# leonsick/depthg

Hardware: AMD Instinct MI355X
Metric: correlation-loss steps/sec at B=32,C=384,28x28 (fwd+bwd, per-GPU batch 32) (higher is better)
Workload: dtype bf16 (feats) / f16 (code) MFMA inputs, f32 accumulate

## Files before the change

### depthg_amd/csrc/dg_api_corr.hip

```cpp
#include "dg_api.h"
#include "dg_corr_args.h"
#include "dg_taps.h"

static unsigned long long* g_prof_span = nullptr;
extern "C" int dg_prof_main_span(void* span) { g_prof_span = static_cast<unsigned long long*>(span); return DG_OK; }

enum class Prep { Small, Dense, General };
enum class Sampler { Plane, ChannelLast };
enum class MainKernel { Small, Corr2, CorrMain };
enum class Depth { None, Job, GsBlocks, GsOwnLaunch };
enum class Hist { Rows, Blobs };
enum class Masks { None, Sampled, DenseRaw, DenseSplit };

struct PairSet {
    int rop;
    int op;
    int neg;
    bool mapped;
    float shift;
    int slot_loss, slot_cd;
    float fin_scale;
    int gidx, csel, dest;
    float factor;
};
// ... 23 lines not shown
    float shift_depth;
    float inv_numel;
    float grad_f, grad_fn;
    int blob, blob_off_c;
    PairSet ps[DG_MAX_NEG + 2];
    Operand ops[DG_MAX_NEG + 2];
    bool gr_on;
    int gr_nkeys, gr_cpb, gr_blocks_per_image;
    int8_t gr_key[DG_MAX_JOBS], gr_first[DG_MAX_JOBS];
    int32_t gr_nblk[DG_MAX_JOBS];
    size_t nhwc_f[2], nhwc_c[2];
    size_t rows_f[DG_MAX_NEG + 2], rows_c[DG_MAX_NEG + 2];
    size_t op[DG_MAX_NEG + 2], inv[DG_MAX_NEG + 2], colpart[DG_MAX_NEG + 2], bbar[DG_MAX_NEG + 2];
    size_t ccolpart[DG_MAX_NEG + 2], csum[DG_MAX_NEG + 2], bsplit[DG_MAX_NEG + 2];
    size_t rvec[DG_MAX_NEG + 2], rimg[DG_MAX_NEG + 2];
    size_t nz, nzsum;
    size_t dRA[DG_MAX_NEG + 3], dRB[DG_MAX_NEG + 2];
    size_t part[DG_MAX_NEG + 3];
    size_t comb[2], scratch_out, taps, gbuf[DG_MAX_NEG + 2];
    size_t ticket;
    size_t maskbits[DG_MAX_NEG + 2];
    size_t clo[2];
    size_t gr_list, gr_count, gr_rank;
    size_t dRA2[DG_MAX_NEG + 2], dRBs[DG_MAX_NEG + 2], dRB2[DG_MAX_NEG + 2][2], dRBm[DG_MAX_NEG + 2], part4, om;
    size_t total;

    bool small() const { return prep == Prep::Small; }
    bool dense() const { return prep == Prep::Dense; }
    bool plane() const { return sampler == Sampler::Plane; }
    bool has_masks() const { return masks != Masks::None; }
    bool depth_in_gs() const { return depth_run == Depth::GsBlocks || depth_run == Depth::GsOwnLaunch; }
    bool dense_masks() const { return masks == Masks::DenseRaw || masks == Masks::DenseSplit; }
    bool intra_symmetric() const { return !pointwise || fold; }
    const int64_t* batch_map(int k, const int64_t* perms) const {
        return k < 0 ? nullptr : reinterpret_cast<const int64_t*>(reinterpret_cast<uintptr_t>(perms) + (size_t)k * B * sizeof(int64_t));
    }
    const int64_t* map_of(int t, const int64_t* perms) const { return batch_map(ps[t].mapped ? ps[t].neg : -1, perms); }
};

static inline float* f32(char* ws, size_t off) { return reinterpret_cast<float*>(ws + off); }

#define FOLD_STASH_OFF (5 * 1024)

static void plan_tables(const dg_corr_desc* d, Plan& p) {
    const double numel = (double)p.B * p.P * p.P;
    p.inv_numel = (float)(1.0 / numel);
// ... 125 lines not shown
    for (int i = 0; i < 2; ++i) p.comb[i] = take(B * p.Ppad * p.KD * 4);
    p.scratch_out = take(DG_OUT_COUNT * 4);
    p.taps = take(2 * B * dg_taps_record_bytes(p.hc * p.wc, p.P));
    for (int t = 0; t < p.T; ++t) p.gbuf[t] = p.grad ? take(B * (size_t)(p.Ppad / 32) * (p.Ppad / 32) * 2048) : 0;
    p.ticket = take(256);
    const bool xmask = rows && !p.small() && p.grad && plain_zero_clamp && p.Ppad <= 256 && p.rf == 4;
    const bool xmask_dense = (d->flags & DG_EXACT_MASKS) && ident && p.grad && plain_zero_clamp &&
                             p.KF == 384 && p.KD == 96 && p.D <= 80 && p.Ppad >= 160 && p.B <= 64;
    if ((d->flags & DG_EXACT_MASKS) && p.grad && (d->flags & DG_ZERO_CLAMP) && !xmask && !xmask_dense && !p.small())
        return fail(DG_ERR_UNSUPPORTED, "DG_EXACT_MASKS: exact clamp masks exist on small sample grids (always on there) and on the dense "
                                        "identity grid with C <= 384 (padded to 384), D <= 80, P >= 160, B <= 64, zero_clamp without stabalize");
    p.masks = xmask ? Masks::Sampled : (!xmask_dense ? Masks::None : (p.pointwise ? Masks::DenseSplit : Masks::DenseRaw));
    for (int t = 0; t < p.T; ++t) p.maskbits[t] = take(p.has_masks() ? B * (size_t)(p.Ppad / 32) * p.Ppad * 4 : 0);
    p.main = p.small() ? MainKernel::Small
                       : (p.grad && dg_corr2_shape_supported(p.KF, p.KD, p.D, p.lo, p.hi, p.Ppad, p.B) ? MainKernel::Corr2 : MainKernel::CorrMain);
    static const bool fold_on = [] { const char* e = getenv("DG_FOLD_INTRA"); return !(e && e[0] == '0'); }();
    p.fold = fold_on && p.main == MainKernel::Corr2 && p.pointwise && !xmask;
    p.half = p.main == MainKernel::Corr2 && ident && p.N * p.B <= 512 && p.S == p.h && p.S == p.w;
    p.depth_run = (!p.depth || p.small()) ? Depth::None : (!p.grad ? Depth::Job : (p.dense_masks() ? Depth::GsOwnLaunch : Depth::GsBlocks));
    for (int i = 0; i < 2; ++i) p.clo[i] = take(p.masks == Masks::DenseSplit ? B * (size_t)(p.Ppad / 32) * p.KD * 64 : 0);
    p.gr_list = take((size_t)DG_MAX_JOBS * B * DG_GR_CAP * 4);
    p.gr_count = take((size_t)DG_MAX_JOBS * B * 4);
    p.gr_rank = take((size_t)DG_MAX_JOBS * B * 2);
    {
        const bool sg = p.small() && p.grad, two = sg && p.pointwise;
        const size_t gt = B * p.Ppad * p.KD * 4;
        for (int t = 0; t < p.T; ++t) {
            p.dRA2[t] = take(two ? gt : 0);
            p.dRBs[t] = take(sg && p.nsplit == 2 ? gt : 0);
            for (int k = 0; k < 2; ++k) p.dRB2[t][k] = take(two && k < p.nsplit ? gt : 0);
            p.dRBm[t] = take(sg && t >= 2 && (p.pointwise || p.nsplit == 2) ? gt : 0);
        }
        p.part4 = take(p.small() ? (size_t)(p.T + 1) * B * p.nsplit * 16 : 0);
        p.om = take(p.small() ? (size_t)(p.T + 1) * 4 : 0);
    }
    if (intra_feats) {
        const int x = p.xop = p.T;
        p.nhwc_x = take(rows ? 0 : B * HW * p.C4 * 4);
        p.rows_f[x] = take(want_rows ? B * p.P * frow : 0); p.rows_c[x] = p.rows_c[0];
        p.op[x] = take(B * (p.Ppad / 32) * (size_t)p.blob);
        p.inv[x] = take(B * p.Ppad * 4);
        p.colpart[x] = take(B * (size_t)(p.Ppad / 32) * p.KF * 4);
        p.bbar[x] = take(B * p.KF * 4);
        p.bsplit[x] = take(B * 2 * p.KF * 2);
        p.ccolpart[x] = take(B * (size_t)(p.Ppad / 32) * p.KD * 4);
        p.csum[x] = take(B * p.KD * 4);
// ... 345 lines not shown
    return DG_OK;
}

static int fwd_colmeans(Fwd& c) {
    const Plan& p = c.p;
    const DgCorrArgs& a = c.a;
    DgColmeanArgs m;
    memset(&m, 0, sizeof(m));
    m.nops = p.nopx(); m.B = p.B; m.P = p.P; m.Ppad = p.Ppad; m.KF = p.KF; m.KD = p.KD;
    for (int o = 0; o < p.nopx(); ++o) {
        m.colpart[o] = p.pointwise ? f32(c.ws, p.colpart[o]) : nullptr; m.bbar[o] = f32(c.ws, p.bbar[o]);
        m.bsplit[o] = reinterpret_cast<__bf16*>(c.ws + p.bsplit[o]);
        m.ngroups[o] = p.Ppad / 32;
        m.ccolpart[o] = f32(c.ws, p.ccolpart[o]); m.csum[o] = f32(c.ws, p.csum[o]);
    }
    m.zero_word = p.depth_in_gs() ? reinterpret_cast<unsigned int*>(c.ws + p.ticket) : nullptr;
    m.zero_words9 = a.wctr;
    if (p.gr_on) {
        m.gr.nh = p.T; m.gr.nkeys = p.gr_nkeys; m.gr.B = p.B;
        for (int t = 0; t < p.T; ++t) { m.gr.sidx[t] = p.map_of(t, c.perms); m.gr.key[t] = p.gr_key[t]; }
        m.gr.list = reinterpret_cast<int32_t*>(c.ws + p.gr_list); m.gr.count = reinterpret_cast<int32_t*>(c.ws + p.gr_count);
        m.gr.rank = reinterpret_cast<int16_t*>(c.ws + p.gr_rank);
    }
    if (p.dense() && p.pointwise) {
        m.dc.code[0] = c.code; m.dc.code[1] = c.code_pos;
        for (int o = 0; o < 2; ++o) { m.dc.blob[o] = c.ws + p.op[o]; m.dc.inv_norm[o] = f32(c.ws, p.inv[o]); m.dc.ccolpart[o] = f32(c.ws, p.ccolpart[o]); }
        m.dc.B = p.B; m.dc.D = p.D; m.dc.KF = p.KF; m.dc.KD = p.KD; m.dc.h = p.h; m.dc.w = p.w; m.dc.P = p.P; m.dc.Ppad = p.Ppad;
        if (p.masks == Masks::DenseSplit) { m.dc.clo[0] = c.ws + p.clo[0]; m.dc.clo[1] = c.ws + p.clo[1]; }
    }
    if (c.split) {
        DgColmeanArgs ms = m;
        ms.zsel = 1; m.zsel = 2;
        DG_HIP(c.side->hand_over(0));
        DG_HIP(dg_launch_colmean(ms, c.side->stream()));
    }
    DG_HIP(dg_launch_colmean(m, c.stream));
    return DG_OK;
}

static int fwd_cd_mask3(Fwd& c) {
    const Plan& p = c.p;
    DgCdMask3Args m;
    memset(&m, 0, sizeof(m));
    m.opR = c.ws + p.op[0]; m.loR = c.ws + p.clo[0];
    for (int t = 0; t < p.T; ++t) {
        m.opS[t] = c.ws + p.op[p.ps[t].op]; m.loS[t] = c.ws + p.clo[p.ps[t].op]; m.sidx[t] = p.map_of(t, c.perms);
// ... 228 lines not shown
static int corr_backward_impl(const dg_corr_desc* desc, const float* grad_scalars, const float* grad_total, const float* coords1,
                              const float* coords2, const int64_t* perms, float* grad_code, float* grad_code_pos,
                              void* workspace, size_t workspace_bytes, dg_stream_t stream_) {
    Plan p{};
    int rc = make_plan(desc, p);
    if (rc != DG_OK) return rc;
    if (!p.grad) return fail(DG_ERR_INVALID, "dg_corr_backward needs a descriptor with DG_NEED_GRAD (as used in forward)");
    if (!coords1 || !coords2 || !grad_code || !grad_code_pos || !workspace) return fail(DG_ERR_INVALID, "null pointer");
    if (p.N > 0 && !perms) return fail(DG_ERR_INVALID, "perms is null with n_neg=%d", p.N);
    if (workspace_bytes < p.total) return fail(DG_ERR_WORKSPACE, "workspace %zu < required %zu bytes", workspace_bytes, p.total);
    char* ws = static_cast<char*>(workspace);
    DgScatterArgs s;
    memset(&s, 0, sizeof(s));
    ScatterFill fill{s, ws};
    if (p.small()) scatter_sources_small(p, perms, fill);
    else scatter_sources_blobs(p, perms, fill);
    if (p.depth) fill.add(p.dRA[p.T], nullptr, 3, 0, 2.0f * p.grad_f, 0, 1);
    s.coords1 = coords1; s.coords2 = coords2; s.gscal = grad_scalars; s.gtot = grad_total;
    s.wtot[0] = desc->w_intra; s.wtot[1] = desc->w_inter; s.wtot[2] = desc->w_neg; s.wtot[3] = desc->w_depth;
    s.comb[0] = f32(ws, p.comb[0]); s.comb[1] = f32(ws, p.comb[1]);
    s.taps = ws + p.taps;
    s.xop = ws + p.op[0]; s.xinv = f32(ws, p.inv[0]); s.blob_bytes = p.blob; s.blob_off_c = p.blob_off_c;
    s.xinv_dest[0] = f32(ws, p.inv[0]); s.xinv_dest[1] = p.nops > 1 ? f32(ws, p.inv[1]) : nullptr;
    s.out[0] = grad_code; s.out[1] = grad_code_pos;
    s.B = p.B; s.D = p.D; s.DP = p.KD; s.h = p.hc; s.w = p.wc; s.S = p.S; s.Sh = p.Sh; s.P = p.P; s.Ppad = p.Ppad;
    if ((size_t)p.hc * p.wc > 4096) return fail(DG_ERR_UNSUPPORTED, "code map %dx%d too large for the gradient gather (max 4096 pixels)", p.hc, p.wc);
    s.DC = 8;
    s.dense = p.dense() ? 1 : 0;
    s.taps_ready = p.dense() ? 0 : 1;
    DG_HIP(dg_launch_scatter(s, static_cast<hipStream_t>(stream_)));
    return DG_OK;
}

extern "C" int dg_corr_backward(const dg_corr_desc* desc, const float* grad_scalars, const float* coords1,
                                const float* coords2, const int64_t* perms, float* grad_code, float* grad_code_pos,
                                void* workspace, size_t workspace_bytes, dg_stream_t stream_) {
    if (!grad_scalars) return fail(DG_ERR_INVALID, "null pointer");
    return corr_backward_impl(desc, grad_scalars, nullptr, coords1, coords2, perms, grad_code, grad_code_pos, workspace,
                              workspace_bytes, stream_);
}

extern "C" int dg_corr_backward_total(const dg_corr_desc* desc, const float* grad_total, const float* coords1,
                                      const float* coords2, const int64_t* perms, float* grad_code, float* grad_code_pos,
                                      void* workspace, size_t workspace_bytes, dg_stream_t stream_) {
    if (!grad_total) return fail(DG_ERR_INVALID, "null pointer");
    return corr_backward_impl(desc, nullptr, grad_total, coords1, coords2, perms, grad_code, grad_code_pos, workspace,
// ... 125 lines not shown
```

### depthg_amd/csrc/dg_corr_args.h

```cpp
#pragma once
#include "dg_device.h"

__host__ __device__ inline int dg_perm32(int pl) {
    int s = pl >> 4, u = (pl >> 3) & 1, hh = (pl >> 2) & 1, v = pl & 3;
    return (2 * s + hh) * 8 + 4 * u + v;
}

#ifndef DG_F_IG
#define DG_F_IG 4
#endif
__host__ __device__ inline int dg_f_off(int q, int g) {
    constexpr int IG = DG_F_IG;
    return ((g / IG) * 32 + q) * (IG * 16) + (((g % IG) ^ ((q / (16 / IG)) % IG)) * 16);
}

struct DgBlob {
    int GF, GD, KD;
    int off_c, off_p, bytes;
    __host__ __device__ DgBlob(int KF, int KD_) : GF(KF / 8), GD(KD_ / 8), KD(KD_) {
        off_c = 32 * GF * 16;
        off_p = off_c + GD * 32 * 16;
        bytes = off_p + 4 * KD * 16;
    }
    __host__ __device__ int f(int q, int g) const { return dg_f_off(q, g); }
// ... 1 lines not shown
    __host__ __device__ int p(int d, int cc) const { return off_p + (cc * KD + d) * 16; }
};

template <int NKF, int NKD>
struct BlobT {
    static constexpr int KF = NKF * 16, KD = NKD * 16, GF = KF / 8, GD = KD / 8;
    static constexpr int OFF_C = 32 * GF * 16;
    static constexpr int OFF_P = OFF_C + GD * 32 * 16;
    static constexpr int BYTES = OFF_P + 4 * KD * 16;
    static constexpr int CHUNKS = BYTES / 1024;
    static constexpr int CHUNK_C0 = OFF_C / 1024;
    static constexpr int CHUNK_P0 = OFF_P / 1024;
    static_assert(BYTES % 1024 == 0 && OFF_C % 1024 == 0 && OFF_P % 1024 == 0, "blob parts must be KiB multiples");
    static_assert(GF % 16 == 0, "swizzle needs 16-granule groups");
};

__host__ __device__ inline size_t dg_gtile_off(int p, int d, int DP) {
    const int q = p & 31;
    return ((size_t)(p >> 5) * (DP >> 5) + (d >> 5)) * 1024 + (q >> 3) * 256 + ((d & 31) + 32 * ((q >> 2) & 1)) * 4 + (q & 3);
}

#define DG_XROWS_LDS (4 * 33 * 16)
template <int NDF>
__device__ __forceinline__ void dg_load_code_rows(const char* Cp, char* T, int lane, _Float16 (&x)[NDF][16]) {
        const int r = lane & 31, h = lane >> 5;
    i32x4 raw[NDF][2];
#pragma unroll
    for (int f = 0; f < NDF; ++f)
#pragma unroll
        for (int k = 0; k < 2; ++k) raw[f][k] = *reinterpret_cast<const i32x4*>(Cp + f * 2048 + k * 1024 + lane * 16);
#pragma unroll
    for (int f = 0; f < NDF; ++f) {
#pragma unroll
        for (int k = 0; k < 2; ++k) {
            const int L = k * 64 + lane;
            *reinterpret_cast<i32x4*>(T + ((L >> 5) * 33 + (L & 31)) * 16) = raw[f][k];
        }
#pragma unroll
        for (int i = 0; i < 16; ++i) {
            const int q = (i & 3) + 8 * (i >> 2) + 4 * h;
            x[f][i] = *reinterpret_cast<const _Float16*>(T + ((r >> 3) * 33 + q) * 16 + (r & 7) * 2);
        }
    }
}

enum { DG_JOB_HELPER = 0, DG_JOB_DEPTH = 1 };

struct DgJob {
    const char* Rop;
    const char* Sop;
    const float* rvec;
    const float* rimg;
    const uint32_t* maskbits;
    const float* nzR;
    const float* nzS;
    const float* RcInv;
    const float* Scsum;
    const int64_t* ridx;
    const int64_t* sidx;
    float* dR;
    float* part;
    float* out_cd;
    float* out_loss;
    uint16_t* Gout;
    float shift;
    int32_t kind;
// ... 251 lines not shown
    const int B = g.B;
    int src[DG_MAX_JOBS];
#pragma unroll
    for (int j = 0; j < DG_MAX_JOBS; ++j) {
        const bool mine = j < g.nh && g.key[j] == key && lane < B;
        const int64_t* sidx = mine ? g.sidx[j] : nullptr;
        src[j] = mine ? (sidx ? (int)sidx[lane] : lane) : -1;
    }
    int cnt = 0;
#pragma unroll
    for (int j = 0; j < DG_MAX_JOBS; ++j) {
        const bool hit = src[j] == m;
        const unsigned long long mask = __ballot(hit);
        if (hit) {
            const int rk = cnt + __popcll(mask & ((1ull << lane) - 1ull));
            g.rank[j * B + lane] = (int16_t)(rk < 32767 ? rk : 32767);
            if (rk < DG_GR_CAP) g.list[(key * B + m) * DG_GR_CAP + rk] = j | (lane << 8);
        }
        cnt += __popcll(mask);
    }
    if (lane == 0) g.count[key * B + m] = cnt < DG_GR_CAP ? cnt : DG_GR_CAP;
}

struct DgColmeanArgs {
    const float* colpart[DG_MAX_NEG + 2];
    float* bbar[DG_MAX_NEG + 2];
    __bf16* bsplit[DG_MAX_NEG + 2];
    const float* ccolpart[DG_MAX_NEG + 2];
    float* csum[DG_MAX_NEG + 2];
    int32_t ngroups[DG_MAX_NEG + 2];
    int32_t nops, B, P, Ppad, KF, KD;
    unsigned int* zero_word;
    unsigned int* zero_words9;
    DgGroupArgs gr;
    DgDenseCodeArgs dc;
    int32_t zsel;
};

struct DgRowmeanJob {
    const char* A;
    const float* bbar;
    const __bf16* bsplit;
    const int64_t* aidx;
    const int64_t* bidx;
    float* rvec;
    float* rimg;
};
struct DgRowmeanArgs {
    DgRowmeanJob jobs[DG_MAX_NEG + 2];
    int32_t njobs, B, P, Ppad, KF, KD;
    const float* abar;
    const char* xA;
    const float* xabar;
    char* stash;
    int32_t stash_off;
    const float* cs_part[2];
    float* cs_out[2];
// ... 14 lines not shown
#define DG_MAX_SCATTER 48
struct DgScatterArgs {
    DgScatterSrc src[DG_MAX_SCATTER];
    int32_t nsrc;
    const float* coords1;
    const float* coords2;
    const float* gscal;
    const float* gtot;
    float wtot[4];
    float* comb[2];
    char* taps;
    const char* xop;
    const float* xinv;
    const float* xinv_dest[2];
    int32_t blob_bytes, blob_off_c;
    float* out[2];
    int32_t B, D, DP, h, w, S, Sh, P, Ppad, DC;
    int32_t dense;
    int8_t craw[2][DG_MAX_SCATTER / 2], cfin[2][DG_MAX_SCATTER / 2];
    int8_t ncraw[2], ncfin[2];
    int8_t crawh[2][DG_MAX_SCATTER / 2], cfinh[2][DG_MAX_SCATTER / 2];
    int8_t ncrawh[2], ncfinh[2];
    int32_t routed_half;
    int32_t taps_ready;
    int32_t naxpy;
    float* axo[DG_MAX_NEG + 2];
    const float* axd[DG_MAX_NEG + 2];
    const float* axd2[DG_MAX_NEG + 2];
    const float* axs[DG_MAX_NEG + 2];
    const float* axs2[DG_MAX_NEG + 2];
    const float* axf[DG_MAX_NEG + 2];
};

__device__ __forceinline__ float dg_src_factor(const DgScatterSrc& q) { return q.dfac ? q.factor * q.dfac[0] : q.factor; }
__device__ __forceinline__ float dg_gscal(const DgScatterArgs& a, int i) {
    return a.gscal ? a.gscal[i] + a.gscal[DG_OUT_TOTAL] * a.wtot[i] : a.gtot[0] * a.wtot[i];
}

struct DgGsJob {
    const uint16_t* G;
    const char* Rop;
    const char* Sop;
    const float* ScInv;
    const int64_t* ridx;
    const int64_t* sidx;
    float* dS;
// ... 66 lines not shown
```

### depthg_amd/csrc/dg_post.hip

```cpp
#include "dg_device.h"
#include "dg_corr_args.h"
#include "dg_taps.h"
#include <cstdlib>

typedef const float __attribute__((address_space(1)))* gfloat_p;


#define DG_LOAD_GS(a, gs)                                                                                   \
    float gs[4];                                                                                            \
    {                                                                                                       \
        const bool vec_ = (a).gscal != nullptr;                                                             \
        const float gt_ = vec_ ? (a).gscal[DG_OUT_TOTAL] : (a).gtot[0];                                     \
        const float g0_ = vec_ ? (a).gscal[0] : 0.f, g1_ = vec_ ? (a).gscal[1] : 0.f;                       \
        const float g2_ = vec_ ? (a).gscal[2] : 0.f, g3_ = vec_ ? (a).gscal[3] : 0.f;                       \
        gs[0] = g0_ + gt_ * (a).wtot[0]; gs[1] = g1_ + gt_ * (a).wtot[1];                                  \
        gs[2] = g2_ + gt_ * (a).wtot[2]; gs[3] = g3_ + gt_ * (a).wtot[3];                                  \
    }
__device__ __forceinline__ float dg_pick(const float (&gs)[4], int i) { return i == 0 ? gs[0] : (i == 1 ? gs[1] : (i == 2 ? gs[2] : gs[3])); }

template <int NDF>
__global__ __launch_bounds__(64 * NDF) void k_grad_combine(const DgScatterArgs a) {
    const int rt = blockIdx.x, n = blockIdx.y, dest = blockIdx.z;
    const int lane = threadIdx.x & 63, r = lane & 31, h = lane >> 5, DP = NDF * 32;
    const int d = __builtin_amdgcn_readfirstlane((int)threadIdx.x >> 6);
    if (dest >= 2) {
        const int j = dest - 2;
        const size_t off = ((size_t)n * (a.Ppad >> 5) + rt) * (32 * DP) + d * 1024 + lane * 4;
        const float f = a.axf[j] ? a.axf[j][0] : 0.f;
// ... 68 lines not shown
            const float inv = rr < a.P ? a.xinv[(size_t)n * a.Ppad + rr] : 0.f;
            v[i] = (v[i] - (float)x[0][i] * t) * inv;
        }
    }
    add_sources(a.cfin[dest], a.ncfin[dest]);
    if (ok) {
        float* out = a.comb[dest] + tile_off;
#pragma unroll
        for (int g = 0; g < 4; ++g) {
            const f32x4 t = {v[4 * g], v[4 * g + 1], v[4 * g + 2], v[4 * g + 3]};
            *reinterpret_cast<f32x4*>(out + g * 256) = t;
        }
    }
}

#ifndef COMB_HB_HM
#define COMB_HB_HM 4
#endif
#ifndef COMB_HB
#define COMB_HB 4
#endif
#define COMB_MAXROUTE 512
template <int NDF, bool HM = false>
__global__ __launch_bounds__(64 * NDF) void k_combine_out(const DgScatterArgs a) {
    const int rt = blockIdx.x, n = blockIdx.y, dest = blockIdx.z;
    const int tid = threadIdx.x, lane = tid & 63, r = lane & 31, h = lane >> 5, DP = NDF * 32;
    const int d = __builtin_amdgcn_readfirstlane(tid >> 6);
    __shared__ __attribute__((aligned(16))) char xs[NDF][DG_XROWS_LDS];
    __shared__ float part[NDF][32];
    __shared__ float stage[NDF][32 * 33];
    __shared__ const float* rl_p[COMB_MAXROUTE];
    __shared__ float rl_w[COMB_MAXROUTE];
    __shared__ int rl_cnt, wcnt[NDF], rsrc[DG_MAX_SCATTER];
    DG_LOAD_GS(a, gs)
    int nr = 0;
    for (int s = 0; s < a.nsrc; ++s)
        if (a.src[s].dest == dest && a.src[s].route != nullptr) { if (tid == 0) rsrc[nr] = s; ++nr; }
    if (tid == 0) rl_cnt = 0;
    __syncthreads();
    for (int i0 = 0; i0 < nr * a.B; i0 += 64 * NDF) {
        const int i = i0 + tid;
        bool hit = false;
        int m = 0, s = 0;
        if (i < nr * a.B) {
            const int rs = i / a.B;
            m = i - rs * a.B; s = rsrc[rs];
            hit = (int)a.src[s].route[m] == n;
        }
        const unsigned long long bal = __ballot(hit);
        if (lane == 0) wcnt[d] = __popcll(bal);
        __syncthreads();
        int base = rl_cnt;
        for (int wv = 0; wv < d; ++wv) base += wcnt[wv];
        if (hit) {
            const int o = base + __popcll(bal & ((1ull << lane) - 1));
            const DgScatterSrc& q = a.src[s];
            if (o < COMB_MAXROUTE) {
                rl_p[o] = q.half ? reinterpret_cast<const float*>(reinterpret_cast<const _Float16*>(q.buf) + (size_t)m * a.Ppad * a.DP) : q.buf + (size_t)m * a.Ppad * a.DP;
                rl_w[o] = dg_src_factor(q) * dg_pick(gs, q.gidx);
            }
        }
        __syncthreads();
        if (tid == 0) {
            int c = rl_cnt;
            for (int wv = 0; wv < NDF; ++wv) c += wcnt[wv];
            rl_cnt = min(c, COMB_MAXROUTE);
        }
        __syncthreads();
    }
    const int cnt = rl_cnt;
    const bool ok = 32 * d + r < a.D;
    const size_t in_img = (size_t)rt * (32 * DP) + lane * 4 + (ok ? d * 1024 : 0);
    const size_t tile_off = (size_t)n * a.Ppad * DP + in_img;
    float v[16];
#pragma unroll
    for (int i = 0; i < 16; ++i) v[i] = 0.f;
    const size_t in_img_h = (size_t)rt * (32 * DP) + lane * 8 + (ok ? d * 1024 : 0);
    constexpr int HB = HM ? COMB_HB_HM : COMB_HB, FB = HM ? 1 : 4;
    float invd[16];
#pragma unroll
    for (int i = 0; i < 16; ++i) {
        const int rr = rt * 32 + (i & 3) + 8 * (i >> 2) + 4 * h;
        invd[i] = (a.xinv_dest[dest] && rr < a.P) ? a.xinv_dest[dest][(size_t)n * a.Ppad + rr] : 0.f;
    }
    const _Float16 __attribute__((address_space(1)))* const hdummy = reinterpret_cast<const _Float16 __attribute__((address_space(1)))*>(reinterpret_cast<uintptr_t>(a.xinv));
    auto add_half4 = [&](const _Float16 __attribute__((address_space(1)))* const (&hb)[HB], const float (&sc)[HB], const bool raw) __attribute__((always_inline)) {
        f16x8 t0[HB], t1[HB];
#pragma unroll
        for (int u = 0; u < HB; ++u) {
            t0[u] = *reinterpret_cast<const f16x8 __attribute__((address_space(1)))*>(hb[u]);
            t1[u] = *reinterpret_cast<const f16x8 __attribute__((address_space(1)))*>(hb[u] + ((ok && hb[u] != hdummy) ? 512 : 0));
        }
#pragma unroll
        for (int u = 0; u < HB; ++u) {
            const bool use = ok && sc[u] != 0.f;
#pragma unroll
            for (int e = 0; e < 8; ++e) {
                v[e] = fmaf(raw ? sc[u] : sc[u] * invd[e], use ? (float)t0[u][e] : 0.f, v[e]);
                v[8 + e] = fmaf(raw ? sc[u] : sc[u] * invd[8 + e], use ? (float)t1[u][e] : 0.f, v[8 + e]);
            }
        }
    };
    auto add_sources_half = [&](const int8_t* list, const int nsrc_, const bool raw) __attribute__((always_inline)) {
        for (int k0 = 0; k0 < nsrc_; k0 += HB) {
            const _Float16 __attribute__((address_space(1)))* hb[HB];
            float sc[HB];
#pragma unroll
            for (int u = 0; u < HB; ++u) {
                const bool live = k0 + u < nsrc_;
                const DgScatterSrc& q = a.src[(int)list[live ? k0 + u : k0]];
                sc[u] = live ? dg_src_factor(q) * dg_pick(gs, q.gidx) : 0.f;
                hb[u] = live ? reinterpret_cast<const _Float16 __attribute__((address_space(1)))*>(reinterpret_cast<uintptr_t>(q.buf)) + (size_t)n * a.Ppad * DP + in_img_h
                             : hdummy;
            }
            add_half4(hb, sc, raw);
        }
    };
    auto add_sources = [&](const int8_t* list, const int nsrc_) __attribute__((always_inline)) {

        for (int k0 = 0; k0 < nsrc_; k0 += FB) {
            f32x4 t[FB][4];
            float sc[FB];
#pragma unroll
            for (int u = 0; u < FB; ++u) {
                const bool live = k0 + u < nsrc_;
                const DgScatterSrc& q = a.src[(int)list[live ? k0 + u : k0]];
                sc[u] = live ? dg_src_factor(q) * dg_pick(gs, q.gidx) : 0.f;
                const float* base = q.buf + tile_off;
#pragma unroll
                for (int g = 0; g < 4; ++g) t[u][g] = *reinterpret_cast<const f32x4*>(base + (ok ? g * 256 : 0));
            }
#pragma unroll
            for (int u = 0; u < FB; ++u) {
                const bool use = ok && k0 + u < nsrc_;
#pragma unroll
                for (int g = 0; g < 4; ++g)
#pragma unroll
                    for (int e = 0; e < 4; ++e) v[4 * g + e] = fmaf(sc[u], use ? t[u][g][e] : 0.f, v[4 * g + e]);
            }
        }
    };
    const int nraw = a.ncraw[dest] + a.ncrawh[dest];
    add_sources(a.craw[dest], a.ncraw[dest]);
    add_sources_half(a.crawh[dest], a.ncrawh[dest], true);
    if (nraw > 0) {
        const char* xb = a.xop + ((size_t)n * (a.Ppad >> 5) + rt) * a.blob_bytes + a.blob_off_c + d * 2048;
        _Float16 x[1][16];
        dg_load_code_rows<1>(xb, xs[d], lane, x);
#pragma unroll
        for (int i = 0; i < 16; ++i) {
            const float t = half_sum((float)x[0][i] * v[i]);
            if (r == 0) part[d][h * 16 + i] = t;
        }
        __syncthreads();
#pragma unroll
        for (int i = 0; i < 16; ++i) {
            float t = part[0][h * 16 + i];
#pragma unroll
            for (int f = 1; f < NDF; ++f) t += part[f][h * 16 + i];
            const int rr = rt * 32 + (i & 3) + 8 * (i >> 2) + 4 * h;
            const float inv = rr < a.P ? a.xinv[(size_t)n * a.Ppad + rr] : 0.f;
            v[i] = (v[i] - (float)x[0][i] * t) * inv;
        }
    }
    add_sources(a.cfin[dest], a.ncfin[dest]);
    add_sources_half(a.cfinh[dest], a.ncfinh[dest], false);
    if (a.routed_half) {
        for (int e0 = 0; e0 < cnt; e0 += HB) {
            const _Float16 __attribute__((address_space(1)))* hb[HB];
            float sc[HB];
#pragma unroll
            for (int k = 0; k < HB; ++k) {
                const int e = min(e0 + k, cnt - 1);
                sc[k] = e0 + k < cnt ? rl_w[e] : 0.f;
                hb[k] = sc[k] != 0.f ? reinterpret_cast<const _Float16 __attribute__((address_space(1)))*>(reinterpret_cast<uintptr_t>(rl_p[e])) + in_img_h : hdummy;
            }
            add_half4(hb, sc, false);
        }
    } else
    for (int e0 = 0; e0 < cnt; e0 += 4) {
        f32x4 u4[4][4];
        float sc[4];
#pragma unroll
        for (int k = 0; k < 4; ++k) {
            const int e = min(e0 + k, cnt - 1);
            sc[k] = e0 + k < cnt ? rl_w[e] : 0.f;
            const gfloat_p sb = (gfloat_p)rl_p[e] + in_img;
#pragma unroll
            for (int g = 0; g < 4; ++g) u4[k][g] = *(const f32x4 __attribute__((address_space(1)))*)(sb + (ok ? g * 256 : 0));
        }
#pragma unroll
        for (int k = 0; k < 4; ++k)
#pragma unroll
            for (int g = 0; g < 4; ++g)
#pragma unroll
                for (int e = 0; e < 4; ++e) v[4 * g + e] = fmaf(sc[k], ok ? u4[k][g][e] : 0.f, v[4 * g + e]);
    }
    float* st = stage[d];
#pragma unroll
    for (int i = 0; i < 16; ++i) st[r * 33 + (i & 3) + 8 * (i >> 2) + 4 * h] = v[i];
    __builtin_amdgcn_fence(__ATOMIC_RELEASE, "workgroup");
    __builtin_amdgcn_wave_barrier();
    __builtin_amdgcn_fence(__ATOMIC_ACQUIRE, "workgroup");
    const int HW = a.h * a.w, p = rt * 32 + r;
    float* out = a.out[dest] + (size_t)n * a.D * HW + p;
#pragma unroll
    for (int it = 0; it < 16; ++it) {
        const int c = 2 * it + h, ch = 32 * d + c;
        if (ch < a.D && p < a.P) out[(size_t)ch * HW] = st[c * 33 + r];
    }
// ... 364 lines not shown
    {
        for (int dest = 0; dest < 2; ++dest) {
            ac.ncraw[dest] = ac.ncfin[dest] = ac.ncrawh[dest] = ac.ncfinh[dest] = 0;
            for (int i = 0; i < a.nsrc; ++i) {
                const DgScatterSrc& q = a.src[i];
                if (q.dest != dest || q.route != nullptr) continue;
                int8_t& cnt = q.half ? (q.raw ? ac.ncrawh[dest] : ac.ncfinh[dest]) : (q.raw ? ac.ncraw[dest] : ac.ncfin[dest]);
                if (cnt >= DG_MAX_SCATTER / 2) return hipErrorInvalidValue;
                (q.half ? (q.raw ? ac.crawh[dest] : ac.cfinh[dest]) : (q.raw ? ac.craw[dest] : ac.cfin[dest]))[cnt++] = (int8_t)i;
            }
        }
        const dim3 cgrid(a.Ppad / 32, a.B, 2);
        {
            int nrouted = 0;
            for (int i = 0; i < a.nsrc; ++i) nrouted += a.src[i].route != nullptr;
            bool any_half = false;
            int routed_h = 0;
            for (int i = 0; i < a.nsrc; ++i) { any_half = any_half || a.src[i].half != 0; routed_h += (a.src[i].route != nullptr && a.src[i].half) ? 1 : 0; }
            if (routed_h != 0 && routed_h != nrouted) return hipErrorInvalidValue;
            ac.routed_half = routed_h != 0 ? 1 : 0;
            const bool one_launch = a.dense && a.S == a.h && a.S == a.w && nrouted * a.B <= COMB_MAXROUTE && (a.DP == 96 || a.DP == 128);
            if (any_half && !one_launch) return hipErrorInvalidValue;
            if (one_launch) {
                if (a.DP == 96 && any_half) hipLaunchKernelGGL((k_combine_out<3, true>), cgrid, dim3(192), 0, s, ac);
                else if (a.DP == 96) hipLaunchKernelGGL(k_combine_out<3>, cgrid, dim3(192), 0, s, ac);
                else hipLaunchKernelGGL(k_combine_out<4>, cgrid, dim3(256), 0, s, ac);
                return hipGetLastError();
            }
        }
        const dim3 cgrid2(a.Ppad / 32, a.B, 2 + a.naxpy);
        if (a.DP == 96) hipLaunchKernelGGL(k_grad_combine<3>, cgrid2, dim3(192), 0, s, ac);
        else if (a.DP == 128) hipLaunchKernelGGL(k_grad_combine<4>, cgrid2, dim3(256), 0, s, ac);
        else return hipErrorInvalidValue;
    }
    const int HW = a.h * a.w;
    {
        int nrouted = 0;
        for (int i = 0; i < a.nsrc; ++i) nrouted += a.src[i].route != nullptr;
        int CGv = 16;
        auto stage_bytes = [&](int cg) { return (size_t)cg * (HW + 2) * 4 + (size_t)DENSE_MAXROUTE * 12; };
        if (stage_bytes(CGv) > 150 * 1024 && CGv > 8) CGv = 8;
        const size_t dsm = stage_bytes(CGv);
        if (a.dense && a.S == a.h && a.S == a.w && dsm <= 150 * 1024 && (size_t)nrouted * a.B <= DENSE_MAXROUTE) {
            auto launch = [&](auto kern, int threads) { return dg_launch(kern, dim3(a.DP / CGv, a.B, 2), dim3(threads), (int)dsm, s, a); };
            if (CGv == 32) return launch(k_scatter_dense<32, 1024>, 1024);
            if (CGv == 16) return launch(k_scatter_dense<16, 512>, 512);
// ... 313 lines not shown
```

### depthg_amd/csrc/dg_prep.hip

```cpp
#include "dg_device.h"
#include "dg_corr_args.h"
#include "dg_taps.h"
#include <cstdlib>

__global__ void k_nchw_to_nhwc(const DgTransposeArgs a) {
    __shared__ float t[32][33];
    const int b = blockIdx.z;
    int m = 0, gy = blockIdx.y;
    while (m < a.nmaps - 1 && gy >= (a.K4[m] + 31) / 32) { gy -= (a.K4[m] + 31) / 32; ++m; }
    const float* __restrict__ src = a.src[m];
    float* __restrict__ dst = a.dst[m];
    const int K = a.K[m], K4 = a.K4[m], HW = a.HW[m];
    const int k0 = gy * 32, p0 = blockIdx.x * 32;
    if (p0 >= HW) return;
    const int tx = threadIdx.x, ty = threadIdx.y;
    for (int i = ty; i < 32; i += 8) {
        int k = k0 + i, p = p0 + tx;
        t[i][tx] = (k < K && p < HW) ? src[((size_t)b * K + k) * HW + p] : 0.f;
    }
    __syncthreads();
    for (int i = ty; i < 32; i += 8) {
        int p = p0 + i, k = k0 + tx;
        if (p < HW && k < K4) dst[((size_t)b * HW + p) * K4 + k] = t[tx][i];
    }
// ... 906 lines not shown
            for (int u = 0; u < 4; ++u) v[u] = cp[(size_t)(t + u) * K];
#pragma unroll
            for (int u = 0; u < 4; ++u) s += v[u];
        }
        for (; t < ngroups; ++t) s += cp[(size_t)t * K];
        out[(size_t)n * K + k] = s * scale;
    }
}

__global__ __launch_bounds__(256) void k_colmean(const DgColmeanArgs a) {
    extern __shared__ __attribute__((aligned(16))) char cm_smem[];
    const int n = blockIdx.x, o = blockIdx.y;
    if (a.zero_word && n == 0 && o == 0 && blockIdx.z == 0 && threadIdx.x == 0) *a.zero_word = 0u;
    if (a.zero_words9 && n == 0 && o == 0 && blockIdx.z == 0 && threadIdx.x < 9) a.zero_words9[threadIdx.x] = 0u;
    auto reduce = [&](const float* part, int ngroups, int K, float scale, float* out) __attribute__((always_inline)) { colsum_reduce(part, n, ngroups, K, scale, out); };
    if (a.zsel == 1 ? blockIdx.z != 3 : (a.zsel == 2 && blockIdx.z == 3)) return;
    if (blockIdx.z == 3) {
        const int GD = a.dc.KD / 8;
        if ((int)blockIdx.y < 2 * GD) dense_code_planes(a.dc, cm_smem, n, (int)blockIdx.y / GD, (int)blockIdx.y % GD);
        return;
    }
    if (blockIdx.z == 2) {
        if ((int)blockIdx.y < a.gr.nkeys && threadIdx.x < 64) dg_group_lists(a.gr, n, o, threadIdx.x);
        return;
    }
    if (o >= a.nops) return;
    if (blockIdx.z == 0 && a.colpart[o]) {
        reduce(a.colpart[o], a.ngroups[o], a.KF, 1.f / (float)a.P, a.bbar[o]);
        __syncthreads();
        for (int k = threadIdx.x; k < a.KF; k += 256) {
            const float v = a.bbar[o][(size_t)n * a.KF + k];
            const __bf16 hi = (__bf16)v;
            a.bsplit[o][((size_t)n * 2) * a.KF + k] = hi;
            a.bsplit[o][((size_t)n * 2 + 1) * a.KF + k] = (__bf16)(v - (float)hi);
        }
    }
    if (blockIdx.z == 1 && a.ccolpart[o] && a.dc.B == 0) reduce(a.ccolpart[o], a.Ppad / 32, a.KD, 1.f, a.csum[o]);
}

hipError_t dg_launch_colmean(const DgColmeanArgs& a, hipStream_t s) {
    int ny = a.gr.nkeys > a.nops ? a.gr.nkeys : a.nops;
    int nz = a.gr.nkeys > 0 ? 3 : 2, smem = 0;
    if (a.dc.B > 0) {
        if (a.nops != 2) return hipErrorInvalidValue;
        ny = max(ny, 2 * (a.dc.KD / 8)); nz = 4; smem = a.dc.Ppad * 16 * ((a.dc.clo[0] || a.dc.clo[1]) ? 2 : 1);
    }
    return dg_launch_if(a.dc.B > 0, k_colmean, dim3(a.B, ny, nz), dim3(256), smem, s, a);
}

#define ROWMEAN_WAVES 4
template <bool XJ = false>
__global__ __launch_bounds__(64 * ROWMEAN_WAVES) void k_rowmean(const DgRowmeanArgs a) {
    extern __shared__ __attribute__((aligned(16))) char rm_smem[];
    const int tile = blockIdx.x, n = blockIdx.y, tid = threadIdx.x, lane = tid & 63, c = lane & 31, h = lane >> 5;
    const int wid = __builtin_amdgcn_readfirstlane(tid >> 6);
    const int KF = a.KF, nt = a.Ppad / 32;
    const bool xz = XJ && blockIdx.z == 1;
    if (tile == nt + 1) {
        if (xz) return;
        for (int o = 0; o < a.ncs; ++o) colsum_reduce(a.cs_part[o], n, nt, a.KD, 1.f, a.cs_out[o]);
        return;
    }
    if (tile == nt) {
        float av[12];
        const float* const abar = xz ? a.xabar : a.abar;
// ... 97 lines not shown
```

Measured before the change: 3331.

## Precompute combine route lists in colmean and prefetch sources in combine_out

```diff
diff --git a/depthg_amd/csrc/dg_api_corr.hip b/depthg_amd/csrc/dg_api_corr.hip
--- a/depthg_amd/csrc/dg_api_corr.hip
+++ b/depthg_amd/csrc/dg_api_corr.hip
@@ -69,6 +69,9 @@
     size_t maskbits[DG_MAX_NEG + 2];
     size_t clo[2];
     size_t gr_list, gr_count, gr_rank;
+    bool routes;
+    int rl_cap;
+    size_t rl_ent, rl_cnt;
     size_t dRA2[DG_MAX_NEG + 2], dRBs[DG_MAX_NEG + 2], dRB2[DG_MAX_NEG + 2][2], dRBm[DG_MAX_NEG + 2], part4, om;
     size_t total;
 
@@ -240,6 +243,10 @@
     p.gr_list = take((size_t)DG_MAX_JOBS * B * DG_GR_CAP * 4);
     p.gr_count = take((size_t)DG_MAX_JOBS * B * 4);
     p.gr_rank = take((size_t)DG_MAX_JOBS * B * 2);
+    p.routes = ident && p.grad && p.N > 0 && p.N * p.B <= 512;
+    p.rl_cap = (int)up((size_t)p.N * B, DG_ROUTE_PAD);
+    p.rl_ent = take(p.routes ? 2 * B * p.rl_cap * 4 : 0);
+    p.rl_cnt = take(p.routes ? 2 * B * 4 : 0);
     {
         const bool sg = p.small() && p.grad, two = sg && p.pointwise;
         const size_t gt = B * p.Ppad * p.KD * 4;
@@ -631,6 +638,14 @@
         m.gr.list = reinterpret_cast<int32_t*>(c.ws + p.gr_list); m.gr.count = reinterpret_cast<int32_t*>(c.ws + p.gr_count);
         m.gr.rank = reinterpret_cast<int16_t*>(c.ws + p.gr_rank);
     }
+    if (p.routes) {
+        for (int t = 0; t < p.T; ++t) {
+            const PairSet& q = p.ps[t];
+            if (q.neg >= 0) m.rt.map[q.dest][m.rt.nr[q.dest]++] = p.batch_map(q.neg, c.perms);
+        }
+        m.rt.B = p.B; m.rt.cap = p.rl_cap;
+        m.rt.ent = reinterpret_cast<int32_t*>(c.ws + p.rl_ent); m.rt.cnt = reinterpret_cast<int32_t*>(c.ws + p.rl_cnt);
+    }
     if (p.dense() && p.pointwise) {
         m.dc.code[0] = c.code; m.dc.code[1] = c.code_pos;
         for (int o = 0; o < 2; ++o) { m.dc.blob[o] = c.ws + p.op[o]; m.dc.inv_norm[o] = f32(c.ws, p.inv[o]); m.dc.ccolpart[o] = f32(c.ws, p.ccolpart[o]); }
@@ -905,6 +920,7 @@
     s.taps = ws + p.taps;
     s.xop = ws + p.op[0]; s.xinv = f32(ws, p.inv[0]); s.blob_bytes = p.blob; s.blob_off_c = p.blob_off_c;
     s.xinv_dest[0] = f32(ws, p.inv[0]); s.xinv_dest[1] = p.nops > 1 ? f32(ws, p.inv[1]) : nullptr;
+    if (p.routes) { s.rl_ent = reinterpret_cast<const int32_t*>(ws + p.rl_ent); s.rl_cnt = reinterpret_cast<const int32_t*>(ws + p.rl_cnt); s.rl_cap = p.rl_cap; }
     s.out[0] = grad_code; s.out[1] = grad_code_pos;
     s.B = p.B; s.D = p.D; s.DP = p.KD; s.h = p.hc; s.w = p.wc; s.S = p.S; s.Sh = p.Sh; s.P = p.P; s.Ppad = p.Ppad;
     if ((size_t)p.hc * p.wc > 4096) return fail(DG_ERR_UNSUPPORTED, "code map %dx%d too large for the gradient gather (max 4096 pixels)", p.hc, p.wc);
diff --git a/depthg_amd/csrc/dg_corr_args.h b/depthg_amd/csrc/dg_corr_args.h
--- a/depthg_amd/csrc/dg_corr_args.h
+++ b/depthg_amd/csrc/dg_corr_args.h
@@ -47,13 +47,15 @@
 
 #define DG_XROWS_LDS (4 * 33 * 16)
 template <int NDF>
-__device__ __forceinline__ void dg_load_code_rows(const char* Cp, char* T, int lane, _Float16 (&x)[NDF][16]) {
-        const int r = lane & 31, h = lane >> 5;
-    i32x4 raw[NDF][2];
+__device__ __forceinline__ void dg_code_rows_issue(const char* Cp, int lane, i32x4 (&raw)[NDF][2]) {
 #pragma unroll
     for (int f = 0; f < NDF; ++f)
 #pragma unroll
         for (int k = 0; k < 2; ++k) raw[f][k] = *reinterpret_cast<const i32x4*>(Cp + f * 2048 + k * 1024 + lane * 16);
+}
+template <int NDF>
+__device__ __forceinline__ void dg_code_rows_turn(const i32x4 (&raw)[NDF][2], char* T, int lane, _Float16 (&x)[NDF][16]) {
+    const int r = lane & 31, h = lane >> 5;
 #pragma unroll
     for (int f = 0; f < NDF; ++f) {
 #pragma unroll
@@ -67,6 +69,12 @@
             x[f][i] = *reinterpret_cast<const _Float16*>(T + ((r >> 3) * 33 + q) * 16 + (r & 7) * 2);
         }
     }
+}
+template <int NDF>
+__device__ __forceinline__ void dg_load_code_rows(const char* Cp, char* T, int lane, _Float16 (&x)[NDF][16]) {
+    i32x4 raw[NDF][2];
+    dg_code_rows_issue<NDF>(Cp, lane, raw);
+    dg_code_rows_turn<NDF>(raw, T, lane, x);
 }
 
 enum { DG_JOB_HELPER = 0, DG_JOB_DEPTH = 1 };
@@ -364,6 +372,32 @@
     if (lane == 0) g.count[key * B + m] = cnt < DG_GR_CAP ? cnt : DG_GR_CAP;
 }
 
+#define DG_ROUTE_PAD 8
+struct DgRouteArgs {
+    const int64_t* map[2][DG_MAX_NEG];
+    int32_t nr[2], B, cap;
+    int32_t* ent;
+    int32_t* cnt;
+};
+__device__ __forceinline__ void dg_route_lists(const DgRouteArgs& g, const int dest, const int n, const int lane) {
+    const int B = g.B, total = g.nr[dest] * B;
+    int32_t* const ent = g.ent + ((size_t)dest * B + n) * g.cap;
+    int cnt = 0;
+    for (int i0 = 0; i0 < total; i0 += 64) {
+        const int i = i0 + lane;
+        int r = 0, m = 0;
+        bool hit = false;
+        if (i < total) {
+            r = i / B; m = i - r * B;
+            hit = (int)g.map[dest][r][m] == n;
+        }
+        const unsigned long long mask = __ballot(hit);
+        if (hit) ent[cnt + __popcll(mask & ((1ull << lane) - 1ull))] = r | (m << 8);
+        cnt += __popcll(mask);
+    }
+    if (lane == 0) g.cnt[dest * B + n] = cnt;
+}
+
 struct DgColmeanArgs {
     const float* colpart[DG_MAX_NEG + 2];
     float* bbar[DG_MAX_NEG + 2];
@@ -375,6 +409,7 @@
     unsigned int* zero_word;
     unsigned int* zero_words9;
     DgGroupArgs gr;
+    DgRouteArgs rt;
     DgDenseCodeArgs dc;
     int32_t zsel;
 };
@@ -435,6 +470,10 @@
     int8_t crawh[2][DG_MAX_SCATTER / 2], cfinh[2][DG_MAX_SCATTER / 2];
     int8_t ncrawh[2], ncfinh[2];
     int32_t routed_half;
+    const int32_t* rl_ent;
+    const int32_t* rl_cnt;
+    int32_t rl_cap;
+    int8_t rsrc[2][DG_MAX_NEG];
     int32_t taps_ready;
     int32_t naxpy;
     float* axo[DG_MAX_NEG + 2];
diff --git a/depthg_amd/csrc/dg_post.hip b/depthg_amd/csrc/dg_post.hip
--- a/depthg_amd/csrc/dg_post.hip
+++ b/depthg_amd/csrc/dg_post.hip
@@ -4,6 +4,7 @@
 #include <cstdlib>
 
 typedef const float __attribute__((address_space(1)))* gfloat_p;
+typedef const _Float16 __attribute__((address_space(1)))* ghalf_p;
 
 
 #define DG_LOAD_GS(a, gs)                                                                                   \
@@ -118,53 +119,21 @@
 #endif
 #define COMB_MAXROUTE 512
 template <int NDF, bool HM = false>
-__global__ __launch_bounds__(64 * NDF) void k_combine_out(const DgScatterArgs a) {
+__global__ __launch_bounds__(64 * NDF) __attribute__((amdgpu_waves_per_eu(HM ? 4 : 3))) void k_combine_out(const DgScatterArgs a) {
     const int rt = blockIdx.x, n = blockIdx.y, dest = blockIdx.z;
     const int tid = threadIdx.x, lane = tid & 63, r = lane & 31, h = lane >> 5, DP = NDF * 32;
     const int d = __builtin_amdgcn_readfirstlane(tid >> 6);
     __shared__ __attribute__((aligned(16))) char xs[NDF][DG_XROWS_LDS];
     __shared__ float part[NDF][32];
     __shared__ float stage[NDF][32 * 33];
-    __shared__ const float* rl_p[COMB_MAXROUTE];
-    __shared__ float rl_w[COMB_MAXROUTE];
-    __shared__ int rl_cnt, wcnt[NDF], rsrc[DG_MAX_SCATTER];
+    constexpr int HB = HM ? COMB_HB_HM : COMB_HB, FB = HM ? 1 : 4;
+    static_assert(HB <= DG_ROUTE_PAD, "the first batch of a route list is read before its count");
     DG_LOAD_GS(a, gs)
-    int nr = 0;
-    for (int s = 0; s < a.nsrc; ++s)
-        if (a.src[s].dest == dest && a.src[s].route != nullptr) { if (tid == 0) rsrc[nr] = s; ++nr; }
-    if (tid == 0) rl_cnt = 0;
-    __syncthreads();
-    for (int i0 = 0; i0 < nr * a.B; i0 += 64 * NDF) {
-        const int i = i0 + tid;
-        bool hit = false;
-        int m = 0, s = 0;
-        if (i < nr * a.B) {
-            const int rs = i / a.B;
-            m = i - rs * a.B; s = rsrc[rs];
-            hit = (int)a.src[s].route[m] == n;
-        }
-        const unsigned long long bal = __ballot(hit);
-        if (lane == 0) wcnt[d] = __popcll(bal);
-        __syncthreads();
-        int base = rl_cnt;
-        for (int wv = 0; wv < d; ++wv) base += wcnt[wv];
-        if (hit) {
-            const int o = base + __popcll(bal & ((1ull << lane) - 1));
-            const DgScatterSrc& q = a.src[s];
-            if (o < COMB_MAXROUTE) {
-                rl_p[o] = q.half ? reinterpret_cast<const float*>(reinterpret_cast<const _Float16*>(q.buf) + (size_t)m * a.Ppad * a.DP) : q.buf + (size_t)m * a.Ppad * a.DP;
-                rl_w[o] = dg_src_factor(q) * dg_pick(gs, q.gidx);
-            }
-        }
-        __syncthreads();
-        if (tid == 0) {
-            int c = rl_cnt;
-            for (int wv = 0; wv < NDF; ++wv) c += wcnt[wv];
-            rl_cnt = min(c, COMB_MAXROUTE);
-        }
-        __syncthreads();
-    }
-    const int cnt = rl_cnt;
+    const int32_t* const ent = a.rl_ent + ((size_t)dest * a.B + n) * a.rl_cap;
+    const int cnt = a.rl_cnt ? min(a.rl_cnt[dest * a.B + n], a.rl_cap) : 0;
+    int ent0[HB];
+#pragma unroll
+    for (int k = 0; k < HB; ++k) ent0[k] = a.rl_cnt ? ent[k] : 0;
     const bool ok = 32 * d + r < a.D;
     const size_t in_img = (size_t)rt * (32 * DP) + lane * 4 + (ok ? d * 1024 : 0);
     const size_t tile_off = (size_t)n * a.Ppad * DP + in_img;
@@ -172,21 +141,33 @@
 #pragma unroll
     for (int i = 0; i < 16; ++i) v[i] = 0.f;
     const size_t in_img_h = (size_t)rt * (32 * DP) + lane * 8 + (ok ? d * 1024 : 0);
-    constexpr int HB = HM ? COMB_HB_HM : COMB_HB, FB = HM ? 1 : 4;
-    float invd[16];
-#pragma unroll
-    for (int i = 0; i < 16; ++i) {
-        const int rr = rt * 32 + (i & 3) + 8 * (i >> 2) + 4 * h;
-        invd[i] = (a.xinv_dest[dest] && rr < a.P) ? a.xinv_dest[dest][(size_t)n * a.Ppad + rr] : 0.f;
-    }
-    const _Float16 __attribute__((address_space(1)))* const hdummy = reinterpret_cast<const _Float16 __attribute__((address_space(1)))*>(reinterpret_cast<uintptr_t>(a.xinv));
-    auto add_half4 = [&](const _Float16 __attribute__((address_space(1)))* const (&hb)[HB], const float (&sc)[HB], const bool raw) __attribute__((always_inline)) {
-        f16x8 t0[HB], t1[HB];
+    const int nraw = a.ncraw[dest] + a.ncrawh[dest];
+    const int prow = rt * 32 + r;
+    const float* const xdp = a.xinv_dest[dest];
+    const float xd = (xdp && prow < a.P) ? xdp[(size_t)n * a.Ppad + prow] : 0.f;
+    const float xi = (nraw > 0 && prow < a.P) ? a.xinv[(size_t)n * a.Ppad + prow] : 0.f;
+    auto row_val = [&](const float x, const int i) __attribute__((always_inline)) { return __shfl(x, (i & 3) + 8 * (i >> 2) + 4 * h, 64); };
+    const ghalf_p hdummy = reinterpret_cast<ghalf_p>(reinterpret_cast<uintptr_t>(a.xinv));
+    auto half_batch = [&](const int8_t* list, const int nsrc_, const int k0, ghalf_p (&hb)[HB], float (&sc)[HB]) __attribute__((always_inline)) {
+#pragma unroll
+        for (int u = 0; u < HB; ++u) {
+            const bool live = k0 + u < nsrc_;
+            const DgScatterSrc& q = a.src[(int)list[live ? k0 + u : k0]];
+            sc[u] = live ? dg_src_factor(q) * dg_pick(gs, q.gidx) : 0.f;
+            hb[u] = live ? reinterpret_cast<ghalf_p>(reinterpret_cast<uintptr_t>(q.buf)) + (size_t)n * a.Ppad * DP + in_img_h : hdummy;
+        }
+    };
+    auto half_load = [&](const ghalf_p (&hb)[HB], f16x8 (&t0)[HB], f16x8 (&t1)[HB]) __attribute__((always_inline)) {
 #pragma unroll
         for (int u = 0; u < HB; ++u) {
             t0[u] = *reinterpret_cast<const f16x8 __attribute__((address_space(1)))*>(hb[u]);
             t1[u] = *reinterpret_cast<const f16x8 __attribute__((address_space(1)))*>(hb[u] + ((ok && hb[u] != hdummy) ? 512 : 0));
         }
+    };
+    auto half_add = [&](const f16x8 (&t0)[HB], const f16x8 (&t1)[HB], const float (&sc)[HB], const bool raw) __attribute__((always_inline)) {
+        float invd[16];
+#pragma unroll
+        for (int i = 0; i < 16; ++i) invd[i] = raw ? 1.f : row_val(xd, i);
 #pragma unroll
         for (int u = 0; u < HB; ++u) {
             const bool use = ok && sc[u] != 0.f;
@@ -197,52 +178,55 @@
             }
         }
     };
-    auto add_sources_half = [&](const int8_t* list, const int nsrc_, const bool raw) __attribute__((always_inline)) {
-        for (int k0 = 0; k0 < nsrc_; k0 += HB) {
-            const _Float16 __attribute__((address_space(1)))* hb[HB];
-            float sc[HB];
-#pragma unroll
-            for (int u = 0; u < HB; ++u) {
-                const bool live = k0 + u < nsrc_;
-                const DgScatterSrc& q = a.src[(int)list[live ? k0 + u : k0]];
-                sc[u] = live ? dg_src_factor(q) * dg_pick(gs, q.gidx) : 0.f;
-                hb[u] = live ? reinterpret_cast<const _Float16 __attribute__((address_space(1)))*>(reinterpret_cast<uintptr_t>(q.buf)) + (size_t)n * a.Ppad * DP + in_img_h
-                             : hdummy;
-            }
-            add_half4(hb, sc, raw);
-        }
-    };
-    auto add_sources = [&](const int8_t* list, const int nsrc_) __attribute__((always_inline)) {
-
-        for (int k0 = 0; k0 < nsrc_; k0 += FB) {
-            f32x4 t[FB][4];
-            float sc[FB];
-#pragma unroll
-            for (int u = 0; u < FB; ++u) {
-                const bool live = k0 + u < nsrc_;
-                const DgScatterSrc& q = a.src[(int)list[live ? k0 + u : k0]];
-                sc[u] = live ? dg_src_factor(q) * dg_pick(gs, q.gidx) : 0.f;
-                const float* base = q.buf + tile_off;
-#pragma unroll
-                for (int g = 0; g < 4; ++g) t[u][g] = *reinterpret_cast<const f32x4*>(base + (ok ? g * 256 : 0));
-            }
-#pragma unroll
-            for (int u = 0; u < FB; ++u) {
-                const bool use = ok && k0 + u < nsrc_;
-#pragma unroll
-                for (int g = 0; g < 4; ++g)
-#pragma unroll
-                    for (int e = 0; e < 4; ++e) v[4 * g + e] = fmaf(sc[u], use ? t[u][g][e] : 0.f, v[4 * g + e]);
-            }
-        }
-    };
-    const int nraw = a.ncraw[dest] + a.ncrawh[dest];
-    add_sources(a.craw[dest], a.ncraw[dest]);
-    add_sources_half(a.crawh[dest], a.ncrawh[dest], true);
-    if (nraw > 0) {
-        const char* xb = a.xop + ((size_t)n * (a.Ppad >> 5) + rt) * a.blob_bytes + a.blob_off_c + d * 2048;
+    auto f32_load = [&](const int8_t* list, const int nsrc_, const int k0, f32x4 (&t)[FB][4], float (&sc)[FB]) __attribute__((always_inline)) {
+#pragma unroll
+        for (int u = 0; u < FB; ++u) {
+            const bool live = k0 + u < nsrc_;
+            const DgScatterSrc& q = a.src[(int)list[live ? k0 + u : k0]];
+            sc[u] = live ? dg_src_factor(q) * dg_pick(gs, q.gidx) : 0.f;
+            const float* base = q.buf + tile_off;
+#pragma unroll
+            for (int g = 0; g < 4; ++g) t[u][g] = *reinterpret_cast<const f32x4*>(base + (ok ? g * 256 : 0));
+        }
+    };
+    auto f32_add = [&](const f32x4 (&t)[FB][4], const float (&sc)[FB], const int nsrc_, const int k0) __attribute__((always_inline)) {
+#pragma unroll
+        for (int u = 0; u < FB; ++u) {
+            const bool use = ok && k0 + u < nsrc_;
+#pragma unroll
+            for (int g = 0; g < 4; ++g)
+#pragma unroll
+                for (int e = 0; e < 4; ++e) v[4 * g + e] = fmaf(sc[u], use ? t[u][g][e] : 0.f, v[4 * g + e]);
+        }
+    };
+    auto routed_batch = [&](const int (&e)[HB], const int e0, ghalf_p (&hb)[HB], float (&sc)[HB]) __attribute__((always_inline)) {
+#pragma unroll
+        for (int k = 0; k < HB; ++k) {
+            const int ek = e0 + k < cnt ? __builtin_amdgcn_readfirstlane(e[k]) : 0;
+            const DgScatterSrc& q = a.src[(int)a.rsrc[dest][ek & 255]];
+            sc[k] = e0 + k < cnt ? dg_src_factor(q) * dg_pick(gs, q.gidx) : 0.f;
+            hb[k] = sc[k] != 0.f ? reinterpret_cast<ghalf_p>(reinterpret_cast<uintptr_t>(q.buf)) + (size_t)(ek >> 8) * a.Ppad * a.DP + in_img_h : hdummy;
+        }
+    };
+    f32x4 tf[FB][4];
+    float scf[FB], sch[HB], scr[HB];
+    ghalf_p hb[HB];
+    f16x8 p0[HB], p1[HB], q0[HB], q1[HB];
+    i32x4 xraw[1][2];
+    if (a.ncraw[dest] > 0) f32_load(a.craw[dest], a.ncraw[dest], 0, tf, scf);
+    if (a.ncrawh[dest] > 0) { half_batch(a.crawh[dest], a.ncrawh[dest], 0, hb, sch); half_load(hb, p0, p1); }
+    for (int k0 = 0; k0 < a.ncraw[dest]; k0 += FB) {
+        if (k0 > 0) f32_load(a.craw[dest], a.ncraw[dest], k0, tf, scf);
+        f32_add(tf, scf, a.ncraw[dest], k0);
+    }
+    if (nraw > 0) dg_code_rows_issue<1>(a.xop + ((size_t)n * (a.Ppad >> 5) + rt) * a.blob_bytes + a.blob_off_c + d * 2048, lane, xraw);
+    for (int k0 = 0; k0 < a.ncrawh[dest]; k0 += HB) {
+        if (k0 > 0) { half_batch(a.crawh[dest], a.ncrawh[dest], k0, hb, sch); half_load(hb, p0, p1); }
+        half_add(p0, p1, sch, true);
+    }
+    auto project = [&]() __attribute__((always_inline)) {
         _Float16 x[1][16];
-        dg_load_code_rows<1>(xb, xs[d], lane, x);
+        dg_code_rows_turn<1>(xraw, xs[d], lane, x);
 #pragma unroll
         for (int i = 0; i < 16; ++i) {
             const float t = half_sum((float)x[0][i] * v[i]);
@@ -254,24 +238,36 @@
             float t = part[0][h * 16 + i];
 #pragma unroll
             for (int f = 1; f < NDF; ++f) t += part[f][h * 16 + i];
-            const int rr = rt * 32 + (i & 3) + 8 * (i >> 2) + 4 * h;
-            const float inv = rr < a.P ? a.xinv[(size_t)n * a.Ppad + rr] : 0.f;
-            v[i] = (v[i] - (float)x[0][i] * t) * inv;
-        }
-    }
-    add_sources(a.cfin[dest], a.ncfin[dest]);
-    add_sources_half(a.cfinh[dest], a.ncfinh[dest], false);
-    if (a.routed_half) {
+            v[i] = (v[i] - (float)x[0][i] * t) * row_val(xi, i);
+        }
+    };
+    const bool routed_h = (HM || a.routed_half) && cnt > 0;
+    const bool early = a.ncfin[dest] + a.ncfinh[dest] == 0;
+    if (early) {
+        if (routed_h) { routed_batch(ent0, 0, hb, scr); half_load(hb, q0, q1); }
+        if (nraw > 0) project();
+    } else {
+        if (nraw > 0) project();
+        for (int k0 = 0; k0 < a.ncfin[dest]; k0 += FB) {
+            f32_load(a.cfin[dest], a.ncfin[dest], k0, tf, scf);
+            f32_add(tf, scf, a.ncfin[dest], k0);
+        }
+        for (int k0 = 0; k0 < a.ncfinh[dest]; k0 += HB) {
+            half_batch(a.cfinh[dest], a.ncfinh[dest], k0, hb, sch);
+            half_load(hb, p0, p1);
+            half_add(p0, p1, sch, false);
+        }
+    }
+    if (HM || a.routed_half) {
         for (int e0 = 0; e0 < cnt; e0 += HB) {
-            const _Float16 __attribute__((address_space(1)))* hb[HB];
-            float sc[HB];
-#pragma unroll
-            for (int k = 0; k < HB; ++k) {
-                const int e = min(e0 + k, cnt - 1);
-                sc[k] = e0 + k < cnt ? rl_w[e] : 0.f;
-                hb[k] = sc[k] != 0.f ? reinterpret_cast<const _Float16 __attribute__((address_space(1)))*>(reinterpret_cast<uintptr_t>(rl_p[e])) + in_img_h : hdummy;
-            }
-            add_half4(hb, sc, false);
+            if (e0 > 0 || !early) {
+                int e[HB];
+#pragma unroll
+                for (int k = 0; k < HB; ++k) e[k] = e0 > 0 ? ent[min(e0 + k, cnt - 1)] : ent0[k];
+                routed_batch(e, e0, hb, scr);
+                half_load(hb, q0, q1);
+            }
+            half_add(q0, q1, scr, false);
         }
     } else
     for (int e0 = 0; e0 < cnt; e0 += 4) {
@@ -279,9 +275,10 @@
         float sc[4];
 #pragma unroll
         for (int k = 0; k < 4; ++k) {
-            const int e = min(e0 + k, cnt - 1);
-            sc[k] = e0 + k < cnt ? rl_w[e] : 0.f;
-            const gfloat_p sb = (gfloat_p)rl_p[e] + in_img;
+            const int ek = __builtin_amdgcn_readfirstlane(ent[min(e0 + k, cnt - 1)]);
+            const DgScatterSrc& q = a.src[(int)a.rsrc[dest][ek & 255]];
+            sc[k] = e0 + k < cnt ? dg_src_factor(q) * dg_pick(gs, q.gidx) : 0.f;
+            const gfloat_p sb = (gfloat_p)q.buf + (size_t)(ek >> 8) * a.Ppad * a.DP + in_img;
 #pragma unroll
             for (int g = 0; g < 4; ++g) u4[k][g] = *(const f32x4 __attribute__((address_space(1)))*)(sb + (ok ? g * 256 : 0));
         }
@@ -692,6 +689,16 @@
             const bool one_launch = a.dense && a.S == a.h && a.S == a.w && nrouted * a.B <= COMB_MAXROUTE && (a.DP == 96 || a.DP == 128);
             if (any_half && !one_launch) return hipErrorInvalidValue;
             if (one_launch) {
+                int nr[2] = {0, 0};
+                for (int i = 0; i < a.nsrc; ++i) {
+                    const DgScatterSrc& q = a.src[i];
+                    if (q.route == nullptr) continue;
+                    if (q.dest < 0 || q.dest > 1 || nr[q.dest] >= DG_MAX_NEG) return hipErrorInvalidValue;
+                    ac.rsrc[q.dest][nr[q.dest]++] = (int8_t)i;
+                }
+                const int nrmax = nr[0] > nr[1] ? nr[0] : nr[1];
+                if (nrouted > 0 && (!a.rl_cnt || !a.rl_ent || a.rl_cap < nrmax * a.B || a.rl_cap % DG_ROUTE_PAD != 0)) return hipErrorInvalidValue;
+                if (a.DP == 96 && any_half && nrouted > 0 && !ac.routed_half) return hipErrorInvalidValue;
                 if (a.DP == 96 && any_half) hipLaunchKernelGGL((k_combine_out<3, true>), cgrid, dim3(192), 0, s, ac);
                 else if (a.DP == 96) hipLaunchKernelGGL(k_combine_out<3>, cgrid, dim3(192), 0, s, ac);
                 else hipLaunchKernelGGL(k_combine_out<4>, cgrid, dim3(256), 0, s, ac);
diff --git a/depthg_amd/csrc/dg_prep.hip b/depthg_amd/csrc/dg_prep.hip
--- a/depthg_amd/csrc/dg_prep.hip
+++ b/depthg_amd/csrc/dg_prep.hip
@@ -952,6 +952,7 @@
     }
     if (blockIdx.z == 2) {
         if ((int)blockIdx.y < a.gr.nkeys && threadIdx.x < 64) dg_group_lists(a.gr, n, o, threadIdx.x);
+        if (a.rt.cnt && o < 2 && threadIdx.x >= 64 && threadIdx.x < 128) dg_route_lists(a.rt, o, n, (int)threadIdx.x - 64);
         return;
     }
     if (o >= a.nops) return;
@@ -970,7 +971,7 @@
 
 hipError_t dg_launch_colmean(const DgColmeanArgs& a, hipStream_t s) {
     int ny = a.gr.nkeys > a.nops ? a.gr.nkeys : a.nops;
-    int nz = a.gr.nkeys > 0 ? 3 : 2, smem = 0;
+    int nz = (a.gr.nkeys > 0 || a.rt.cnt) ? 3 : 2, smem = 0;
     if (a.dc.B > 0) {
         if (a.nops != 2) return hipErrorInvalidValue;
         ny = max(ny, 2 * (a.dc.KD / 8)); nz = 4; smem = a.dc.Ppad * 16 * ((a.dc.clo[0] || a.dc.clo[1]) ? 2 : 1);
```

Result: no change. 3359, median of 3 (+0.8%).
